# ratt-ru/pfb-clean

Measured on AMD Instinct MI355X. Metric: PCG matvecs/sec (FFT-conv A^H A apply), 4k x 4k x 8-band cube, higher is better.
Workload: dtype f32; 1 GPU; 4096x4096x8-band cube PCG (hessian_psf + Tikhonov, M = x/sigmainv, tol=0, minit=maxit=20); nx_psf=8192, bands_per_gpu=8, parallelism=band-shard x1, allreduce_hook=False

## Files before the change

pfb_clean_amd/csrc/fft_pow2.hpp:

```cpp
#pragma once
#include "common.hpp"
#include <type_traits>

namespace pfb {

constexpr int ilog2(int n) { return n <= 1 ? 0 : 1 + ilog2(n >> 1); }
constexpr int imin(int a, int b) { return a < b ? a : b; }

constexpr int rmax_of(int E) { return E < 16 ? E : 16; }

template <int N, int E, int P> struct PassRadix { static constexpr int R = imin(rmax_of(E), N / P); };

template <int N, int E, int P>
struct PtwOffset {
    static constexpr int RM = rmax_of(E);
    static constexpr int prev = P / RM;
    static constexpr int value = (P <= RM) ? 0 : PtwOffset<N, E, (P / RM < 1 ? 1 : P / RM)>::value + 4 * prev;
};
template <int N, int E> struct PtwOffset<N, E, 1> { static constexpr int value = 0; };

template <int N, int E>
constexpr int ptw_total() {
    int tot = 0;
    for (int P = rmax_of(E); P < N; P *= rmax_of(E)) tot += 4 * P;
// ... 59 lines not shown

template <typename T, bool INV, int m>
__device__ __forceinline__ cplx<T> mul_w16(cplx<T> a) {
    constexpr T c = T(0.92387953251128675612818318939678828682L);
    constexpr T s = T(0.38268343236508977172845998403039886676L);
    constexpr T h = T(0.70710678118654752440084436210484903928L);
    constexpr int mm = m & 15;
    if constexpr (mm == 0) return a;
    else if constexpr (mm == 4) return rot90<T, INV>(a);
    else if constexpr (mm == 8) return cplx<T>(-a.x, -a.y);
    else if constexpr (mm == 12) return rot90<T, !INV>(a);
    else if constexpr (mm == 2)  return h * (INV ? mul_1pi(a) : mul_1mi(a));
    else if constexpr (mm == 14) return h * (INV ? mul_1mi(a) : mul_1pi(a));
    else if constexpr (mm == 6)  return (-h) * (INV ? mul_1mi(a) : mul_1pi(a));
    else if constexpr (mm == 10) return (-h) * (INV ? mul_1pi(a) : mul_1mi(a));
    else {
        constexpr T wr = (mm == 1) ? c : (mm == 3) ? s : (mm == 5) ? -s : (mm == 7) ? -c : (mm == 9) ? -c
                       : (mm == 11) ? -s : (mm == 13) ? s : c;
        constexpr T wi = (mm == 1) ? s : (mm == 3) ? c : (mm == 5) ? c : (mm == 7) ? s : (mm == 9) ? -s
                       : (mm == 11) ? -c : (mm == 13) ? -c : -s;
        const T wy = INV ? wi : -wi;
        return a * cplx<T>(wr, wy);
    }
}

template <typename T, bool INV, int R> struct Dft;

template <typename T, bool INV> struct Dft<T, INV, 2> {
    __device__ __forceinline__ static void run(cplx<T> (&u)[2]) { dft2<T, INV>(u[0], u[1]); }
};
template <typename T, bool INV> struct Dft<T, INV, 4> {
    __device__ __forceinline__ static void run(cplx<T> (&u)[4]) { dft4<T, INV>(u[0], u[1], u[2], u[3]); }
};
template <typename T, bool INV> struct Dft<T, INV, 8> {
    __device__ __forceinline__ static void run(cplx<T> (&u)[8]) {
        dft4<T, INV>(u[0], u[2], u[4], u[6]);
        dft4<T, INV>(u[1], u[3], u[5], u[7]);
        u[3] = mul_w16<T, INV, 2>(u[3]);
        u[7] = mul_w16<T, INV, 6>(u[7]);
        cplx<T> x[8];
#pragma unroll
        for (int k1 = 0; k1 < 4; ++k1) {
            const cplx<T> p = u[2 * k1], q = u[2 * k1 + 1];
            if (k1 == 2) {
                x[k1] = addrot<INV>(p, q);
                x[k1 + 4] = addrot<!INV>(p, q);
            } else {
                x[k1] = p + q;
                x[k1 + 4] = p - q;
            }
        }
#pragma unroll
        for (int k = 0; k < 8; ++k) u[k] = x[k];
    }
};
template <typename T, bool INV> struct Dft<T, INV, 16> {
    __device__ __forceinline__ static void run(cplx<T> (&u)[16]) {
        dft4<T, INV>(u[0], u[4], u[8], u[12]);
        dft4<T, INV>(u[1], u[5], u[9], u[13]);
        dft4<T, INV>(u[2], u[6], u[10], u[14]);
        dft4<T, INV>(u[3], u[7], u[11], u[15]);
        u[5] = mul_w16<T, INV, 1>(u[5]);   u[6] = mul_w16<T, INV, 2>(u[6]);   u[7] = mul_w16<T, INV, 3>(u[7]);
        u[9] = mul_w16<T, INV, 2>(u[9]);   u[10] = mul_w16<T, INV, 4>(u[10]); u[11] = mul_w16<T, INV, 6>(u[11]);
        u[13] = mul_w16<T, INV, 3>(u[13]); u[14] = mul_w16<T, INV, 6>(u[14]); u[15] = mul_w16<T, INV, 9>(u[15]);
        dft4<T, INV>(u[0], u[1], u[2], u[3]);
        dft4<T, INV>(u[4], u[5], u[6], u[7]);
        dft4<T, INV>(u[8], u[9], u[10], u[11]);
        dft4<T, INV>(u[12], u[13], u[14], u[15]);
        cplx<T> t;
        t = u[1];  u[1] = u[4];   u[4] = t;
        t = u[2];  u[2] = u[8];   u[8] = t;
        t = u[3];  u[3] = u[12];  u[12] = t;
        t = u[6];  u[6] = u[9];   u[9] = t;
        t = u[7];  u[7] = u[13];  u[13] = t;
        t = u[11]; u[11] = u[14]; u[14] = t;
    }
};

struct NoPassHook {
    template <typename K> __device__ __forceinline__ void operator()(K) const {}
};
template <int K> using PassIdx = std::integral_constant<int, K>;

template <typename T, int N, int E, bool WAVE = false, int DBOFF = 0, bool SQTW = false, bool SEQX = false>
struct RegFft {
    static_assert((N & (N - 1)) == 0 && (E & (E - 1)) == 0 && N >= E, "power-of-two sizes");
    static_assert(!WAVE || N / E <= 64, "wave-local exchange needs the group inside one wave");
    __device__ __forceinline__ static void sync() {
        if constexpr (WAVE) __builtin_amdgcn_fence(__ATOMIC_ACQ_REL, "wavefront");
        else __syncthreads();
    }
    static constexpr int TPB = N / E;
    static constexpr int RM = rmax_of(E);
    static constexpr int LDS_ELEMS = N + N / (RM < (128 / (int)sizeof(cplx<T>)) ? RM : (128 / (int)sizeof(cplx<T>)));
    static constexpr int PTW = ptw_total<N, E>();
    static constexpr int PTWC = ptw_total<N, E>() / 4;

    __device__ __forceinline__ static int pad(int i) { return i + (i >> 4); }
    static constexpr int cpad(int c) { return c + (c >> 4); }

    static constexpr int CB = (int)sizeof(cplx<T>);
    static constexpr int SLOTS = 128 / CB;
    template <int P, int R>
    static constexpr int cxpad(int c) {
        if (P == 1) return c + c / SLOTS;
        if (P >= SLOTS) return c;
        return c + (c / (P * R)) * P;
    }
    template <int P, int R>
    __device__ __forceinline__ static int xpad(int c) { return cxpad<P, R>(c); }

    template <bool INV, int P>
    __device__ __forceinline__ static void butterflies(cplx<T> (&v)[E], int t, const cplx<T>* __restrict__ ptw) {
        constexpr int R = PassRadix<N, E, P>::R;
        constexpr int NB = E / R;
#pragma unroll
        for (int q = 0; q < NB; ++q) {
            cplx<T> u[R];
#pragma unroll
            for (int r = 0; r < R; ++r) u[r] = v[q + r * NB];
            if constexpr (P > 1) {
                const int k = (t + TPB * q) & (P - 1);
                const cplx<T>* tb = ptw + (SQTW ? PtwOffset<N, E, P>::value / 4 : PtwOffset<N, E, P>::value) + k;
                cplx<T> w1 = tb[0], w2, w4, w8;
                if constexpr (SQTW) {
                    if constexpr (R > 2) w2 = w1 * w1;
                    if constexpr (R > 4) w4 = w2 * w2;
                    if constexpr (R > 8) w8 = w4 * w4;
                } else {
                    if constexpr (R > 2) w2 = tb[P];
                    if constexpr (R > 4) w4 = tb[2 * P];
                    if constexpr (R > 8) w8 = tb[3 * P];
                }
                auto tw = [](cplx<T> a, cplx<T> w) { return INV ? mulc(a, w) : a * w; };
                u[1] = tw(u[1], w1);
                if constexpr (R > 2) {
                    u[2] = tw(u[2], w2);
                    const cplx<T> w3 = w1 * w2;
                    u[3] = tw(u[3], w3);
                    if constexpr (R > 4) {
                        u[4] = tw(u[4], w4);
                        const cplx<T> w7 = w3 * w4;
                        u[7] = tw(u[7], w7);
                        if constexpr (R > 8) { u[11] = tw(u[11], w3 * w8); u[15] = tw(u[15], w7 * w8); }
                        const cplx<T> w5 = w1 * w4;
                        u[5] = tw(u[5], w5);
                        if constexpr (R > 8) u[13] = tw(u[13], w5 * w8);
                        const cplx<T> w6 = w2 * w4;
                        u[6] = tw(u[6], w6);
                        if constexpr (R > 8) {
                            u[14] = tw(u[14], w6 * w8);
                            u[8] = tw(u[8], w8);
                            u[9] = tw(u[9], w1 * w8);
                            u[10] = tw(u[10], w2 * w8);
                            u[12] = tw(u[12], w4 * w8);
                        }
                    }
                }
            }
            Dft<T, INV, R>::run(u);
#pragma unroll
            for (int r = 0; r < R; ++r) v[q + r * NB] = u[r];
        }
    }

    template <bool INV, int P, int NV, int XCH = 0, int K = 0, typename Hook = NoPassHook>
    __device__ __forceinline__ static void pass(cplx<T> (&v)[NV][E], cplx<T>* lds_in, int t,
                                                const cplx<T>* __restrict__ ptw, const Hook& hook = Hook()) {
        constexpr int R = PassRadix<N, E, P>::R;
        constexpr int NB = E / R;
        hook(PassIdx<K>{});
#pragma unroll
        for (int n = 0; n < NV; ++n) butterflies<INV, P>(v[n], t, ptw);
        if constexpr (P * R < N) {
            cplx<T>* lds = (DBOFF > 0 && (XCH & 1) == 0) ? lds_in + DBOFF : lds_in;
            if constexpr (SEQX) {
#pragma unroll
                for (int n = 0; n < NV; ++n) {
                    sync();
#pragma unroll
                    for (int q = 0; q < NB; ++q) {
                        const int i = t + TPB * q;
                        const int k = i & (P - 1);
                        cplx<T>* wp = lds + xpad<P, R>((i - k) * R + k);
#pragma unroll
                        for (int s = 0; s < R; ++s) wp[cxpad<P, R>(s * P)] = v[n][q + s * NB];
                    }
                    sync();
                    const cplx<T>* rp = lds + xpad<P, R>(t);
#pragma unroll
                    for (int j = 0; j < E; ++j) v[n][j] = rp[cxpad<P, R>(TPB * j)];
                }
            } else {
            if constexpr (DBOFF == 0) sync();
#pragma unroll
            for (int q = 0; q < NB; ++q) {
                const int i = t + TPB * q;
                const int k = i & (P - 1);
                cplx<T>* wp = lds + xpad<P, R>((i - k) * R + k);
#pragma unroll
                for (int n = 0; n < NV; ++n) {
#pragma unroll
                    for (int s = 0; s < R; ++s) wp[n * LDS_ELEMS + cxpad<P, R>(s * P)] = v[n][q + s * NB];
                }
            }
            sync();
            const cplx<T>* rp = lds + xpad<P, R>(t);
#pragma unroll
            for (int n = 0; n < NV; ++n) {
#pragma unroll
                for (int j = 0; j < E; ++j) v[n][j] = rp[n * LDS_ELEMS + cxpad<P, R>(TPB * j)];
            }
            }
            pass<INV, P * R, NV, XCH + 1, K + 1, Hook>(v, lds_in, t, ptw, hook);
        }
    }

    template <bool INV, int NV, int X0 = 0, typename Hook = NoPassHook>
    __device__ __forceinline__ static void runN(cplx<T> (&v)[NV][E], cplx<T>* lds, int t,
                                                const cplx<T>* __restrict__ ptw, const Hook& hook = Hook()) {
        pass<INV, 1, NV, X0, 0, Hook>(v, lds, t, ptw, hook);
    }
    template <int P = 1> static constexpr int nxch() {
        constexpr int R = PassRadix<N, E, P>::R;
        if constexpr (P * R < N) return 1 + nxch<P * R>();
        else return 0;
    }
    static constexpr int NPASS = nxch<1>() + 1;
    template <bool INV, typename Hook = NoPassHook>
    __device__ __forceinline__ static void run(cplx<T> (&v)[E], cplx<T>* lds, int t,
                                               const cplx<T>* __restrict__ ptw, const Hook& hook = Hook()) {
        pass<INV, 1, 1, 0, 0, Hook>(reinterpret_cast<cplx<T>(&)[1][E]>(v), lds, t, ptw, hook);
    }
};

}
```

pfb_clean_amd/csrc/fftconv_pow2.hip:

```cpp
#include "conv_plan.hpp"
#include "fft_pow2.hpp"
#include <vector>
#include <cstdlib>

#ifndef PFB_POW2_PART
#define PFB_POW2_PART 0
#endif
#define PFB_POW2_COL  (PFB_POW2_PART != 1)
#define PFB_POW2_REST (PFB_POW2_PART != 2)

namespace pfb {

#ifndef PFB_STAMP
#define PFB_STAMP 0
#endif
#if PFB_STAMP
#define PFB_STAMP_ITS 4
#define PFB_STAMP_FIRST 2
static __device__ unsigned long long* g_stamp_buf = nullptr;
#define STAMP(KID, it, slot)                                                                              \
    do {                                                                                                  \
        const unsigned _si = (unsigned)((it) - PFB_STAMP_FIRST);                                          \
        if (threadIdx.x == 0 && g_stamp_buf && _si < PFB_STAMP_ITS && blockIdx.x < 1024)                  \
            g_stamp_buf[(((size_t)(KID) * 1024 + blockIdx.x) * PFB_STAMP_ITS + _si) * 16 + (slot)] = wall_clock64(); \
    } while (0)
#else
#define STAMP(KID, it, slot) do { (void)(it); } while (0)
#endif

template <typename T> struct FastCfg;
template <> struct FastCfg<float>  { static constexpr int ECOL = 8; static constexpr int EROWMAX = 32; static constexpr int WCOL = 4; static constexpr int NVB = 2; };
template <> struct FastCfg<double> { static constexpr int ECOL = 8; static constexpr int EROWMAX = 16; static constexpr int WCOL = 2; static constexpr int NVB = 1; };

template <typename T, int L, int E, int GMAX> constexpr int row_groups();
template <typename T, int L, bool INVK> struct RowCfg {
    static constexpr int EMAX = sizeof(T) == 4 ? (INVK ? (L == 4096 ? 16 : 8) : 16) : 8;
    static constexpr int E = (L / 64 < 8) ? 8 : (L / 64 > EMAX ? EMAX : L / 64);
    static constexpr int TPB = L / E;
    static constexpr bool WAVE = TPB <= 64;
    static constexpr int GMAX = INVK ? 4 : 8;
};
template <typename T, int L> struct InvDb {
    using C = RowCfg<T, L, true>;
    static constexpr int G = row_groups<T, L, C::E, C::GMAX>();
    static constexpr int STRIDE = RegFft<T, L, C::E>::LDS_ELEMS + 4;
    static constexpr bool ON = (size_t)(2 * G * STRIDE + L) * sizeof(cplx<T>) + 384 <= (size_t)152 * 1024;
    static constexpr int OFF = ON ? G * STRIDE : 0;
};

constexpr int LDS_BUDGET = 152 * 1024;

constexpr int COL_E4_MAXH = 1024;
template <typename T, int H> constexpr int ecol() { return (H >= 8192 && sizeof(T) == 8) ? 16 : (H <= COL_E4_MAXH && H >= 64 ? 4 : FastCfg<T>::ECOL); }

template <typename T, int L, int E, int GMAX>
constexpr int row_groups() {
    constexpr int TPB = L / E;
    int G = 256 / TPB > GMAX ? 256 / TPB : GMAX;
    const int stride = RegFft<T, L, E>::LDS_ELEMS + 4;
    while (G > 1 && (G * TPB > 1024 || (size_t)G * stride * sizeof(cplx<T>) + 384 > LDS_BUDGET)) G /= 2;
    return G;
}
template <int H, int E>
constexpr int col_groups() { return (H / E) >= 256 ? 1 : 256 / (H / E); }
constexpr int ECOLX = 8;

template <typename T, int NVB> struct alignas(16) Blk { cplx<T> c[NVB]; };
template <typename T, int NVB>
__device__ __forceinline__ Blk<T, NVB> loadb(const cplx<T>* src) {
    return *reinterpret_cast<const Blk<T, NVB>*>(src);
}
template <typename T, int NVB>
__device__ __forceinline__ Blk<T, NVB> loadb_nt(const cplx<T>* src) {
    typedef float v4f __attribute__((ext_vector_type(4)));
    static_assert(sizeof(Blk<T, NVB>) == 16, "16-byte blocks");
    const v4f v = __builtin_nontemporal_load(reinterpret_cast<const v4f*>(src));
    Blk<T, NVB> b;
    __builtin_memcpy(&b, &v, 16);
    return b;
}

template <typename T, int NVB>
__device__ __forceinline__ void storeb(cplx<T>* dst, const Blk<T, NVB>& b) {
    *reinterpret_cast<Blk<T, NVB>*>(dst) = b;
}

template <typename P>
__device__ __forceinline__ P* opaque(P* p) {
    asm volatile("" : "+v"(p));
    return p;
}

__device__ __forceinline__ int launder(int v) {
    asm volatile("" : "+v"(v));
    return v;
}

template <typename T>
__device__ __forceinline__ cplx<T> root32(int k) {
    constexpr T C[9] = {T(1), T(0.98078528040323044912618223613423903697L), T(0.92387953251128675612818318939678828682L),
                        T(0.83146961230254523707878837761790575673L), T(0.70710678118654752440084436210484903928L),
                        T(0.55557023301960222474283081394853287438L), T(0.38268343236508977172845998403039886676L),
                        T(0.19509032201612826784828486847702224093L), T(0)};
    auto cs = [&](int q) -> T {
        q &= 31;
        return q <= 8 ? C[q] : q <= 16 ? -C[16 - q] : q <= 24 ? -C[q - 16] : C[32 - q];
    };
    return cplx<T>(cs(k), -cs(k - 8));
}

template <int G>
__device__ __forceinline__ int xcd_row_group(int bx, int nbx) {
    constexpr int SH = 8 / G;
    if constexpr (SH > 1) {
        if (nbx % (8 * SH) == 0) {
            const int q = bx / (8 * SH), rem = bx % (8 * SH);
            return SH * (q * 8 + (rem & 7)) + (rem >> 3);
        }
    }
    return bx;
}

struct FastDims {
    int nx, ny, M;
    size_t T_band, psf_band;
    size_t xpitch, xband;
};

__host__ __device__ inline void block_of_bin(int v, int L, int nvb, int* blk, int* c) {
    const int m = v >> 1;
    const int nbe = (L + nvb) / nvb;
    *blk = ((v & 1) ? nbe : 0) + m / nvb;
    *c = m % nvb;
}
inline int fast_nblocks(int L, int nvb) { return (L + nvb) / nvb + L / nvb; }
__host__ __device__ inline size_t psf_off(int blk, int u, int c, int H, int nvb, int four) {
// ... 195 lines not shown
        const cplx<T>* c0 = col_of(act ? item : 0);
#pragma unroll
        for (int j = 0; j < E; ++j) {
            if (act) an[j] = loadb<T, NVB>(c0 + NVB * TPB * j);
            else {
#pragma unroll
                for (int c = 0; c < NVB; ++c) an[j].c[c] = cplx<T>(0, 0);
            }
        }
        {
            const cplx<T>* pe0 = psf_of(act ? item : 0);
#pragma unroll
            for (int j = 0; j < E; ++j) q[j] = NT ? loadb_nt<T, NVB>(pe0 + NVB * TPB * j) : loadb<T, NVB>(pe0 + NVB * TPB * j);
        }
    }
    __syncthreads();
#pragma unroll 1
    for (int it = 0; it < niter; ++it, item = item_of(it)) {
        STAMP(1, it, 0);
        const bool active = item < nitems;
        cplx<T>* col = col_of(active ? item : 0);
        const cplx<T>* pe = psf_of(active ? item : 0);
        const cplx<T>* po = pe + (size_t)H * NVB;
        const int nxt = item_of(it + 1);
        const bool nact = nxt < nitems;
        const cplx<T>* cn = col_of(nact ? nxt : (active ? item : 0));
        const cplx<T>* pen = psf_of(nact ? nxt : (active ? item : 0));
        cplx<T> vv[NVB][E], aw[NVB][E];
#pragma unroll
        for (int j = 0; j < E; ++j) {
#pragma unroll
            for (int c = 0; c < NVB; ++c) { vv[c][j] = an[j].c[c]; aw[c][j] = vv[c][j] * tw[j]; }
        }
        auto ld_an = [&](auto k, int base) {
            constexpr int K = decltype(k)::value;
            constexpr int CNT = E / 2;
#pragma unroll
            for (int j = (K * CNT) / NP; j < ((K + 1) * CNT) / NP; ++j)
                an[base + j] = loadb<T, NVB>(cn + NVB * TPB * (base + j));
        };
        STAMP(1, it, 1);
        F::template runN<false, NVB, 0>(vv, lds, t, ltw, [&](auto k) { ld_an(k, 0); });
        STAMP(1, it, 2);
#pragma unroll
        for (int j = 0; j < E; ++j) {
#pragma unroll
            for (int c = 0; c < NVB; ++c) vv[c][j] = vv[c][j] * q[j].c[c];
        }
        STAMP(1, it, 3);
        F::template runN<true, NVB, X1>(vv, lds, t, ltw, [&](auto k) {
            constexpr int K = decltype(k)::value;
#pragma unroll
            for (int j = (K * E) / NP; j < ((K + 1) * E) / NP; ++j) q[j] = NT ? loadb_nt<T, NVB>(po + NVB * TPB * j) : loadb<T, NVB>(po + NVB * TPB * j);
        });
        STAMP(1, it, 4);
        cplx<T> ev[NVB][E];
#pragma unroll
        for (int j = 0; j < E; ++j) {
#pragma unroll
            for (int c = 0; c < NVB; ++c) { ev[c][j] = vv[c][j]; vv[c][j] = aw[c][j]; }
        }
        F::template runN<false, NVB, 0>(vv, lds, t, ltw, [&](auto k) { ld_an(k, E / 2); });
        STAMP(1, it, 5);
#pragma unroll
        for (int j = 0; j < E; ++j) {
#pragma unroll
            for (int c = 0; c < NVB; ++c) vv[c][j] = vv[c][j] * q[j].c[c];
        }
        STAMP(1, it, 6);
        F::template runN<true, NVB, X1>(vv, lds, t, ltw, [&](auto k) {
            constexpr int K = decltype(k)::value;
#pragma unroll
            for (int j = (K * E) / NP; j < ((K + 1) * E) / NP; ++j) q[j] = NT ? loadb_nt<T, NVB>(pen + NVB * TPB * j) : loadb<T, NVB>(pen + NVB * TPB * j);
        });
        STAMP(1, it, 7);
        if (active) {
#pragma unroll
            for (int j = 0; j < E; ++j) {
                Blk<T, NVB> o;
#pragma unroll
                for (int c = 0; c < NVB; ++c) o.c[c] = ev[c][j] + mulc(vv[c][j], tw[j]);
                storeb<T, NVB>(col + NVB * TPB * j, o);
            }
        }
        STAMP(1, it, 8);
    }
}

template <typename T, int H, int E>
struct ColX {
    static constexpr int HS = H / 2;
    using F = RegFft<T, HS, E, false, 0, true>;
    static constexpr int NVB = FastCfg<T>::NVB;
    static constexpr int GC = col_groups<HS, E>();
    static constexpr int NT = GC * F::TPB;
    static constexpr int XB = NVB * F::LDS_ELEMS;
    static constexpr int PTWP = (F::PTWC + 1) & ~1;
    static constexpr size_t LDS = sizeof(cplx<T>) * ((size_t)PTWP + F::TPB + (size_t)GC * XB + (size_t)NT * E * NVB);
    static_assert(E == 8, "root32: the twiddle constants are the 4E-th roots of unity");
};

template <typename T, int H, int E, bool NT = false>
__global__ void __launch_bounds__((ColX<T, H, E>::NT), 2)
k_col_pow2x(cplx<T>* __restrict__ Tw, const cplx<T>* __restrict__ psf_l,
            const cplx<T>* __restrict__ twP, const cplx<T>* __restrict__ ptwc,
            int nblk, int nitems, size_t T_band, size_t psf_band, int band0, int bstep) {
    using X = ColX<T, H, E>;
    using F = typename X::F;
    constexpr int NVB = X::NVB, HS = X::HS, TPB = F::TPB, GC = X::GC, NP = F::NPASS, NTH = X::NT;
    extern __shared__ __attribute__((aligned(16))) char smem[];
    const int g = threadIdx.x / TPB, t = threadIdx.x % TPB;
    cplx<T>* ltw = reinterpret_cast<cplx<T>*>(smem);
    cplx<T>* ltx = ltw + X::PTWP;
    cplx<T>* lds = ltx + TPB + (size_t)g * X::XB;
    Blk<T, NVB>* park = reinterpret_cast<Blk<T, NVB>*>(ltx + TPB + (size_t)GC * X::XB) + threadIdx.x;
    const int stride = gridDim.x * GC;
    const int niter = (nitems + stride - 1) / stride;

    for (int k = threadIdx.x; k < F::PTWC; k += NTH) ltw[k] = ptwc[k];
    for (int k = threadIdx.x; k < TPB; k += NTH) ltx[k] = twP[k];

    auto col_of = [&](int item) -> cplx<T>* {
        const int bl = item / nblk, blk = item - bl * nblk;
        return Tw + (size_t)(band0 + bstep * bl) * T_band + ((size_t)blk * H + t) * NVB;
    };
    auto psf_of = [&](int item) -> const cplx<T>* {
        const int bl = item / nblk, blk = item - bl * nblk;
        return psf_l + (size_t)(band0 + bstep * bl) * psf_band + ((size_t)blk * 2 * H + t) * NVB;
    };
    auto ldq = [&](const cplx<T>* p) __attribute__((always_inline)) { return NT ? loadb_nt<T, NVB>(p) : loadb<T, NVB>(p); };

    int item = blockIdx.x * GC + g;
    Blk<T, NVB> al[E], ah[E], q[E];
    {
        const bool act = item < nitems;
        const cplx<T>* c0 = col_of(act ? item : 0);
#pragma unroll
        for (int j = 0; j < E; ++j) {
            al[j] = loadb<T, NVB>(c0 + NVB * TPB * j);
            ah[j] = loadb<T, NVB>(c0 + NVB * (HS + TPB * j));
        }
    }
    __syncthreads();
#pragma unroll 1
    for (int it = 0; it < niter; ++it, item += stride) {
        const bool active = item < nitems;
        cplx<T>* col = col_of(active ? item : 0);
        const cplx<T>* ps = psf_of(active ? item : 0);
        const int nxt = item + stride;
        const bool nact = nxt < nitems;
        const cplx<T>* cn = col_of(nact ? nxt : (active ? item : 0));
        cplx<T> vv[NVB][E], ol[NVB][E];
        auto wt = [&]() __attribute__((always_inline)) { return ltx[launder(t)]; };
        auto mulq = [&]() __attribute__((always_inline)) {
#pragma unroll
            for (int j = 0; j < E; ++j) {
#pragma unroll
                for (int c = 0; c < NVB; ++c) vv[c][j] = vv[c][j] * q[j].c[c];
            }
        };
        auto qslice = [&](auto k, const cplx<T>* pq) __attribute__((always_inline)) {
            constexpr int K = decltype(k)::value;
#pragma unroll
            for (int j = (K * E) / NP; j < ((K + 1) * E) / NP; ++j) q[j] = ldq(pq + NVB * TPB * j);
        };
        auto fft_q = [&](const cplx<T>* pq) __attribute__((always_inline)) {
// ... 1088 lines not shown
    void* ptw_col;
    void* ptwc_col;
    void* ptw_row;
    void* ptw_row_inv;
    void* ptw_row_inv_p;
    void* twM;
    void* ptwc_row_fwd;
    int num_cu;
    void* ptwc_col_x;
    int col_x;
};
int pow2_col_set_attr(int dtype, int H);
int pow2_col_launch(pfb_conv_plan* p, const FastTables* ft, int band0, int nb, hipStream_t st);
int pow2_col_fwd_launch(pfb_conv_plan* p, const FastTables* ft, const void* Tq, int band, hipStream_t st);

#if PFB_POW2_REST
template <typename T, int N, int E>
static int upload_ptw(void** dev) {
    constexpr int n = ptw_total<N, E>();
    std::vector<cplx<T>> h(n > 0 ? n : 1);
    if (n > 0) fill_ptw<T, N, E>(h.data());
    PFB_HIP_CHECK(hipMalloc(dev, sizeof(cplx<T>) * h.size()));
    PFB_HIP_CHECK(hipMemcpy(*dev, h.data(), sizeof(cplx<T>) * h.size(), hipMemcpyHostToDevice));
    return PFB_OK;
}

template <typename T, int N, int E>
static int prep_ptw(void** dev) { return upload_ptw<T, N, E>(dev); }

template <typename T, int N, int E>
static int prep_ptw_compact(void** dev) {
    constexpr int n = ptw_total<N, E>() / 4;
    std::vector<cplx<T>> h(n > 0 ? n : 1);
    if (n > 0) fill_ptw_compact<T, N, E>(h.data());
    PFB_HIP_CHECK(hipMalloc(dev, sizeof(cplx<T>) * h.size()));
    PFB_HIP_CHECK(hipMemcpy(*dev, h.data(), sizeof(cplx<T>) * h.size(), hipMemcpyHostToDevice));
    return PFB_OK;
}

template <typename T, int L>
static int set_invp_attr() {
    constexpr int E = InvPE<T, L>::E;
    if constexpr (InvP<T, L, E>::OK) {
#define PFB_INVATTR(MODE, BM)                                                                           \
        PFB_HIP_CHECK(hipFuncSetAttribute((const void*)(k_row_inv_pow2p<T, L, E, MODE, BM>),             \
                                          hipFuncAttributeMaxDynamicSharedMemorySize, 160 * 1024))
        PFB_INVATTR(0, false); PFB_INVATTR(1, false); PFB_INVATTR(2, false);
        PFB_INVATTR(0, true);  PFB_INVATTR(1, true);  PFB_INVATTR(2, true);
        if constexpr (inv_pb_ok<T, L, E>()) {
            PFB_HIP_CHECK(hipFuncSetAttribute((const void*)(k_row_inv_pow2p<T, L, E, 2, false, true>),
                                              hipFuncAttributeMaxDynamicSharedMemorySize, 160 * 1024));
            PFB_HIP_CHECK(hipFuncSetAttribute((const void*)(k_row_inv_pow2p<T, L, E, 2, true, true>),
                                              hipFuncAttributeMaxDynamicSharedMemorySize, 160 * 1024));
        }
#undef PFB_INVATTR
    }
    return PFB_OK;
}

template <typename T, int L>
static int prep_fwdp(void** table) {
    if constexpr (FwdP<T, L>::OK) {
        int rc = prep_ptw_compact<T, L, FwdP<T, L>::EOK>(table);
        if (rc != PFB_OK) return rc;
        PFB_HIP_CHECK(hipFuncSetAttribute((const void*)(k_row_fwd_pow2q<T, L, false>),
                                          hipFuncAttributeMaxDynamicSharedMemorySize, 160 * 1024));
        PFB_HIP_CHECK(hipFuncSetAttribute((const void*)(k_row_fwd_pow2q<T, L, true>),
                                          hipFuncAttributeMaxDynamicSharedMemorySize, 160 * 1024));
    } else {
        PFB_HIP_CHECK(hipFuncSetAttribute((const void*)k_row_fwd_pow2<T, L, RowCfg<T, L, false>::E>,
                                          hipFuncAttributeMaxDynamicSharedMemorySize, 160 * 1024));
    }
    return PFB_OK;
}


template <typename T>
static int prep_tables(pfb_conv_plan* p, FastTables* ft) {
    const int H = p->nx, L = p->ny / 2;
    int rc = PFB_ERR_UNSUPPORTED;
    constexpr int lds_max = 160 * 1024;
    switch (H) {
#define X(NN) case NN: rc = prep_ptw<T, NN, ecol<T, NN>()>(&ft->ptw_col);                          \
        if (rc == PFB_OK) rc = prep_ptw_compact<T, NN, ecol<T, NN>()>(&ft->ptwc_col);             \
        if (rc == PFB_OK && NN == 8192) rc = prep_ptw_compact<T, 4096, ECOLX>(&ft->ptwc_col_x);         \
        if (rc == PFB_OK) rc = pow2_col_set_attr(p->dtype, NN); break;
        PFB_POW2_SIZES(X)
#undef X
        default: break;
    }
    if (rc != PFB_OK) return rc;
    rc = PFB_ERR_UNSUPPORTED;
    switch (L) {
#define X(NN) case NN: rc = prep_ptw<T, NN, RowCfg<T, NN, false>::E>(&ft->ptw_row);                   \
        if (rc == PFB_OK) rc = prep_ptw_compact<T, NN, RowCfg<T, NN, true>::E>(&ft->ptw_row_inv);    \
        if (rc == PFB_OK) { if (InvPE<T, NN>::E != RowCfg<T, NN, true>::E) rc = prep_ptw_compact<T, NN, InvPE<T, NN>::E>(&ft->ptw_row_inv_p); \
                            else ft->ptw_row_inv_p = ft->ptw_row_inv; }                            \
        if (rc == PFB_OK) PFB_HIP_CHECK(hipFuncSetAttribute((const void*)k_row_inv_pow2<T, NN, RowCfg<T, NN, true>::E>, \
            hipFuncAttributeMaxDynamicSharedMemorySize, lds_max));                                   \
        if (rc == PFB_OK) rc = set_invp_attr<T, NN>();                                               \
        if (rc == PFB_OK) rc = prep_fwdp<T, NN>(&ft->ptwc_row_fwd); break;
        PFB_POW2_SIZES(X)
#undef X
        default: break;
    }
    if (rc != PFB_OK) return rc;
    std::vector<cplx<T>> h(L);
    const long double two_pi = 6.283185307179586476925286766559005768L;
    for (int n = 0; n < L; ++n) {
        long double a = two_pi * (long double)n / (long double)p->ny;
        h[n] = cplx<T>((T)cosl(a), (T)(-sinl(a)));
    }
    PFB_HIP_CHECK(hipMalloc(&ft->twM, sizeof(cplx<T>) * L));
    PFB_HIP_CHECK(hipMemcpy(ft->twM, h.data(), sizeof(cplx<T>) * L, hipMemcpyHostToDevice));
    return PFB_OK;
}

template <typename T, int L>
static int rows_per_wg() { return row_groups<T, L, RowCfg<T, L, true>::E, RowCfg<T, L, true>::GMAX>(); }

bool pow2_supported(const pfb_conv_plan* p) {
    if (!is_pow2(p->nx) || !is_pow2(p->ny)) return false;
    if (p->P != 2 * p->nx || p->Q != 2 * p->ny) return false;
    if (p->nx < 64 || p->nx > 8192) return false;
    if (p->ny < 128 || p->ny > (p->dtype == PFB_F32 ? 16384 : 8192)) return false;
    return true;
}

int pow2_rows_per_wg(const pfb_conv_plan* p) {
    const int L = p->ny / 2;
    const bool f32 = p->dtype == PFB_F32;
    switch (L) {
#define X(NN) case NN: return f32 ? rows_per_wg<float, NN>() : rows_per_wg<double, NN>();
        PFB_POW2_SIZES(X)
#undef X
        default: return 0;
    }
}

int pow2_nblocks(const pfb_conv_plan* p) {
    return fast_nblocks(p->ny / 2, p->dtype == PFB_F32 ? FastCfg<float>::NVB : FastCfg<double>::NVB);
}
int pow2_nvb(const pfb_conv_plan* p) {
    return p->dtype == PFB_F32 ? FastCfg<float>::NVB : FastCfg<double>::NVB;
}

int pow2_prepare(pfb_conv_plan* p) {
    FastTables* ft = (FastTables*)calloc(1, sizeof(FastTables));
    PFB_REQUIRE(ft != nullptr, PFB_ERR_ALLOC, "pow2_prepare: host alloc failed");
    p->fast_tables = ft;
    int dev = 0;
    hipDeviceProp_t prop;
    if (hipGetDevice(&dev) == hipSuccess && hipGetDeviceProperties(&prop, dev) == hipSuccess)
        ft->num_cu = prop.multiProcessorCount;
    if (ft->num_cu <= 0) ft->num_cu = 256;
    ft->col_x = p->nx >= 8192 ? 1 : 0;
    return p->dtype == PFB_F32 ? prep_tables<float>(p, ft) : prep_tables<double>(p, ft);
}

void pow2_release(pfb_conv_plan* p) {
    FastTables* ft = (FastTables*)p->fast_tables;
    if (!ft) return;
    if (ft->ptw_col) (void)hipFree(ft->ptw_col);
    if (ft->ptwc_col) (void)hipFree(ft->ptwc_col);
    if (ft->ptwc_col_x) (void)hipFree(ft->ptwc_col_x);
    if (ft->ptw_row) (void)hipFree(ft->ptw_row);
    if (ft->ptw_row_inv_p && ft->ptw_row_inv_p != ft->ptw_row_inv) (void)hipFree(ft->ptw_row_inv_p);
// ... 19 lines not shown
int pow2_set_psfhat(pfb_conv_plan* p, const void* psfhat, hipStream_t st) {
    return p->dtype == PFB_F32 ? set_psfhat_t<float>(p, psfhat, st) : set_psfhat_t<double>(p, psfhat, st);
}

template <typename T, int L>
static void launch_row_fwd(pfb_conv_plan* p, const FastTables* ft, void* Tbuf, int band0, int nb, const void* x,
                           const void* beam, size_t xpitch, size_t xband, hipStream_t st);

template <typename T>
static int set_psf_t(pfb_conv_plan* p, const void* psf, void* psfhat_out, hipStream_t st) {
    const FastTables* ft = (const FastTables*)p->fast_tables;
    const int nx = p->nx, ny = p->ny, P = p->P, Q = p->Q, L = ny / 2;
    void* Tq = nullptr;
    if (hipMalloc(&Tq, sizeof(cplx<T>) * 4 * p->T_elems_per_band) != hipSuccess) {
        set_error("pow2_set_psf: device allocation failed (%zu B)", sizeof(cplx<T>) * 4 * p->T_elems_per_band);
        return PFB_ERR_ALLOC;
    }
    int rc = PFB_OK;
    for (int band = 0; band < p->nband && rc == PFB_OK; ++band) {
        const T* pb = (const T*)psf + (size_t)band * P * Q;
        for (int q = 0; q < 4; ++q) {
            const int a = q >> 1, b = q & 1;
            const T* src = pb + (size_t)((1 - a) * nx) * Q + (size_t)(1 - b) * ny;
            switch (L) {
#define X(NN) case NN: launch_row_fwd<T, NN>(p, ft, Tq, q, 1, src, nullptr, (size_t)Q, (size_t)0, st); break;
                PFB_POW2_SIZES(X)
#undef X
                default: set_error("pow2_set_psf: unsupported ny"); rc = PFB_ERR_UNSUPPORTED; break;
            }
        }
        if (rc == PFB_OK) rc = pow2_col_fwd_launch(p, ft, Tq, band, st);
    }
    if (rc == PFB_OK && psfhat_out) {
        const int nv = p->M + 1;
        dim3 grid((nv + 31) / 32, (P + 31) / 32, p->nband);
        hipLaunchKernelGGL((k_unrelayout_psf_pow2<T>), grid, dim3(256), 0, st, (const cplx<T>*)p->psf_l,
                           (cplx<T>*)psfhat_out, P, nv, L, FastCfg<T>::NVB, p->psf_elems_per_band, ft->col_x);
    }
    if (rc == PFB_OK && (hipGetLastError() != hipSuccess || hipStreamSynchronize(st) != hipSuccess)) {
        set_error("pow2_set_psf: kernel launch failed");
        rc = PFB_ERR_HIP;
    }
    (void)hipFree(Tq);
    return rc;
}

int pow2_set_psf(pfb_conv_plan* p, const void* psf, void* psfhat_out, hipStream_t st) {
    return p->dtype == PFB_F32 ? set_psf_t<float>(p, psf, psfhat_out, st) : set_psf_t<double>(p, psf, psfhat_out, st);
}

#endif

#if PFB_POW2_COL
template <typename T, int H>
static void launch_col(pfb_conv_plan* p, const FastTables* ft, int band0, int nb, hipStream_t st) {
    constexpr int E = ecol<T, H>();
    using F = RegFft<T, H, E>;
    constexpr int GC = col_groups<H, E>();
    const int nblk = fast_nblocks(p->ny / 2, FastCfg<T>::NVB);
    const int band_first = band0 + nb - 1;
    const bool psf_nt = sizeof(cplx<T>) * p->psf_elems_per_band * (size_t)nb >= ((size_t)200 << 20);
    if constexpr (H == 8192) {
        if (ft->col_x) {
            using CX = ColX<T, H, ECOLX>;
            using FX = typename CX::F;
            constexpr int GX = CX::GC;
            const int nitems = nblk * nb;
            const int wg_lds = (int)(((size_t)160 * 1024) / CX::LDS);
            int wg_per_cu = (8 * 64) / (GX * FX::TPB) > 0 ? (8 * 64) / (GX * FX::TPB) : 1;
            if (wg_per_cu > wg_lds) wg_per_cu = wg_lds > 0 ? wg_lds : 1;
            const int need = (nitems + GX - 1) / GX;
            const int grid = need < ft->num_cu * wg_per_cu ? need : ft->num_cu * wg_per_cu;
            const size_t ldsx = CX::LDS;
#define PFB_COLX(NTV)                                                                                          \
            hipLaunchKernelGGL((k_col_pow2x<T, H, ECOLX, NTV>), dim3(grid), dim3(GX * FX::TPB), ldsx, st,      \
                               (cplx<T>*)p->T, (const cplx<T>*)p->psf_l, (const cplx<T>*)p->twP,               \
                               (const cplx<T>*)ft->ptwc_col_x, nblk, nitems, p->T_elems_per_band,              \
                               p->psf_elems_per_band, band_first, -1)
            if (psf_nt) PFB_COLX(true); else PFB_COLX(false);
#undef PFB_COLX
            return;
        }
    }
    constexpr size_t lds = sizeof(cplx<T>) * (size_t)GC * FastCfg<T>::NVB * F::LDS_ELEMS;
    constexpr size_t tab = sizeof(cplx<T>) * (size_t)((F::PTWC + 1) & ~1);
    if constexpr (H >= 2048 && lds + tab <= (size_t)160 * 1024) {
        const int nitems = nblk * nb;
        constexpr int wg_per_cu = (8 * 64) / (GC * F::TPB) > 0 ? (8 * 64) / (GC * F::TPB) : 1;
        const int need = (nitems + GC - 1) / GC;
        const int grid = balanced_grid(need, ft->num_cu * wg_per_cu);
        constexpr bool db = wg_per_cu == 1 && 2 * lds + tab <= (size_t)160 * 1024;
#define PFB_COLP(NTV)                                                                                          \
        hipLaunchKernelGGL((k_col_pow2p<T, H, E, db, NTV>), dim3(grid), dim3(GC * F::TPB), (db ? 2 : 1) * lds + tab, st, \
                           (cplx<T>*)p->T, (const cplx<T>*)p->psf_l, (const cplx<T>*)p->twP,                   \
                           (const cplx<T>*)ft->ptwc_col, nblk, nitems, p->T_elems_per_band,                    \
                           p->psf_elems_per_band, band_first, -1)
        if (psf_nt) PFB_COLP(true); else PFB_COLP(false);
#undef PFB_COLP
        return;
    }
    hipLaunchKernelGGL((k_col_pow2<T, H, E>), dim3((nblk + GC - 1) / GC, nb), dim3(GC * F::TPB), lds, st,
                       (cplx<T>*)p->T, (const cplx<T>*)p->psf_l, (const cplx<T>*)p->twP,
                       (const cplx<T>*)ft->ptw_col, nblk, p->T_elems_per_band, p->psf_elems_per_band, band0);
}

template <typename T, int H>
static int col_set_attr() {
    constexpr int lds_max = 160 * 1024;
    constexpr int E = ecol<T, H>();
    PFB_HIP_CHECK(hipFuncSetAttribute((const void*)(k_col_pow2<T, H, E>), hipFuncAttributeMaxDynamicSharedMemorySize, lds_max));
    PFB_HIP_CHECK(hipFuncSetAttribute((const void*)(k_col_fwd_pow2<T, H, E>), hipFuncAttributeMaxDynamicSharedMemorySize, lds_max));
    using F = RegFft<T, H, E>;
    constexpr int GC = col_groups<H, E>();
    constexpr size_t lds = sizeof(cplx<T>) * (size_t)GC * FastCfg<T>::NVB * F::LDS_ELEMS;
    constexpr size_t tab = sizeof(cplx<T>) * (size_t)((F::PTWC + 1) & ~1);
    if constexpr (H >= 2048 && lds + tab <= (size_t)160 * 1024) {
        constexpr int wg_per_cu = (8 * 64) / (GC * F::TPB) > 0 ? (8 * 64) / (GC * F::TPB) : 1;
        constexpr bool db = wg_per_cu == 1 && 2 * lds + tab <= (size_t)160 * 1024;
        PFB_HIP_CHECK(hipFuncSetAttribute((const void*)(k_col_pow2p<T, H, E, db, false>), hipFuncAttributeMaxDynamicSharedMemorySize, lds_max));
        PFB_HIP_CHECK(hipFuncSetAttribute((const void*)(k_col_pow2p<T, H, E, db, true>), hipFuncAttributeMaxDynamicSharedMemorySize, lds_max));
    }
    if constexpr (H == 8192 || (H == 4096 && sizeof(T) == 8)) {
        PFB_HIP_CHECK(hipFuncSetAttribute((const void*)(k_col_pow2x<T, H, ECOLX, false>), hipFuncAttributeMaxDynamicSharedMemorySize, lds_max));
        PFB_HIP_CHECK(hipFuncSetAttribute((const void*)(k_col_pow2x<T, H, ECOLX, true>), hipFuncAttributeMaxDynamicSharedMemorySize, lds_max));
    }
    return PFB_OK;
}
template <typename T>
static int col_set_attr_t(int H) {
    switch (H) {
#define X(NN) case NN: return col_set_attr<T, NN>();
        PFB_POW2_SIZES(X)
#undef X
        default: set_error("pow2: unsupported nx"); return PFB_ERR_UNSUPPORTED;
    }
}
int pow2_col_set_attr(int dtype, int H) {
    return dtype == PFB_F32 ? col_set_attr_t<float>(H) : col_set_attr_t<double>(H);
}
template <typename T>
static int col_launch_t(pfb_conv_plan* p, const FastTables* ft, int band0, int nb, hipStream_t st) {
    switch (p->nx) {
#define X(NN) case NN: launch_col<T, NN>(p, ft, band0, nb, st); break;
        PFB_POW2_SIZES(X)
#undef X
        default: set_error("pow2_apply: unsupported nx"); return PFB_ERR_UNSUPPORTED;
    }
    return PFB_OK;
}
int pow2_col_launch(pfb_conv_plan* p, const FastTables* ft, int band0, int nb, hipStream_t st) {
    return p->dtype == PFB_F32 ? col_launch_t<float>(p, ft, band0, nb, st) : col_launch_t<double>(p, ft, band0, nb, st);
}
template <typename T, int H>
static void launch_col_fwd(pfb_conv_plan* p, const FastTables* ft, const void* Tq, int band, hipStream_t st) {
    constexpr int E = ecol<T, H>();
    using F = RegFft<T, H, E>;
    constexpr int GC = col_groups<H, E>();
    constexpr int NVB = FastCfg<T>::NVB;
    const int L = p->ny / 2;
    const int nblk = fast_nblocks(L, NVB), nbe = (L + NVB) / NVB;
    const size_t lds = sizeof(cplx<T>) * (size_t)GC * NVB * F::LDS_ELEMS;
    hipLaunchKernelGGL((k_col_fwd_pow2<T, H, E>), dim3((nblk + GC - 1) / GC), dim3(GC * F::TPB), lds, st,
                       (const cplx<T>*)Tq, (cplx<T>*)p->psf_l + (size_t)band * p->psf_elems_per_band,
                       (const cplx<T>*)p->twP, (const cplx<T>*)ft->ptw_col, nblk, nbe, p->T_elems_per_band, ft->col_x);
}
template <typename T>
static int col_fwd_launch_t(pfb_conv_plan* p, const FastTables* ft, const void* Tq, int band, hipStream_t st) {
    switch (p->nx) {
#define X(NN) case NN: launch_col_fwd<T, NN>(p, ft, Tq, band, st); break;
        PFB_POW2_SIZES(X)
#undef X
        default: set_error("pow2_set_psf: unsupported nx"); return PFB_ERR_UNSUPPORTED;
    }
    return PFB_OK;
}
int pow2_col_fwd_launch(pfb_conv_plan* p, const FastTables* ft, const void* Tq, int band, hipStream_t st) {
    return p->dtype == PFB_F32 ? col_fwd_launch_t<float>(p, ft, Tq, band, st) : col_fwd_launch_t<double>(p, ft, Tq, band, st);
}
#endif

#if PFB_POW2_REST

template <typename T, int L>
static void launch_row_fwd(pfb_conv_plan* p, const FastTables* ft, void* Tbuf, int band0, int nb, const void* x,
                           const void* beam, size_t xpitch, size_t xband, hipStream_t st) {
    FastDims d{p->nx, p->ny, p->M, p->T_elems_per_band, p->psf_elems_per_band, xpitch, xband};
    if constexpr (FwdP<T, L>::OK) {
        using FP = FwdP<T, L>;
        const int tiles_per_band = p->nx / FP::G, ntiles = tiles_per_band * nb;
        const int grid = ntiles < ft->num_cu * FP::WG_PER_CU ? ntiles : ft->num_cu * FP::WG_PER_CU;
        const long double a = 6.283185307179586476925286766559005768L / (2.0L * (long double)p->ny);
        const cplx<T> wq1((T)cosl(a), (T)(-sinl(a)));
#define PFB_FWDQ(BM)                                                                                              \
        hipLaunchKernelGGL((k_row_fwd_pow2q<T, L, BM>), dim3(grid), dim3(FP::NT), FP::LDS, st, (const T*)x,      \
                           (const T*)beam, (cplx<T>*)Tbuf, (const cplx<T>*)ft->twM,                              \
                           (const cplx<T>*)ft->ptwc_row_fwd, d, band0, tiles_per_band, ntiles, wq1)
        if (beam) PFB_FWDQ(true); else PFB_FWDQ(false);
#undef PFB_FWDQ
    } else {
// ... 128 lines not shown
```

Before: 437.5 cube-matvecs/s.

## Add single-column-per-thread column FFT-conv kernel for f32 4096-point columns

Adds a new column kernel for f32 with H=4096. Each thread pair splits the two interleaved 8-byte columns of a 16-byte block, so every thread handles one column with E=16 instead of a two-column register block. An LDS stride parameter lets the shared exchange interleave both columns, and the kernel uses double-buffered LDS, prefetches the next item's column and PSF data inside the FFT passes, and computes per-element twiddles from a 32nd-root table. The intent is to cut register pressure and raise occupancy, with more latency hidden by prefetching. The cost is more threads per block and narrower 8-byte global accesses in place of 16-byte ones.

```diff
diff --git a/pfb_clean_amd/csrc/fft_pow2.hpp b/pfb_clean_amd/csrc/fft_pow2.hpp
--- a/pfb_clean_amd/csrc/fft_pow2.hpp
+++ b/pfb_clean_amd/csrc/fft_pow2.hpp
@@ -165,7 +165,7 @@
 };
 template <int K> using PassIdx = std::integral_constant<int, K>;
 
-template <typename T, int N, int E, bool WAVE = false, int DBOFF = 0, bool SQTW = false, bool SEQX = false>
+template <typename T, int N, int E, bool WAVE = false, int DBOFF = 0, bool SQTW = false, bool SEQX = false, int LSTR = 1>
 struct RegFft {
     static_assert((N & (N - 1)) == 0 && (E & (E - 1)) == 0 && N >= E, "power-of-two sizes");
     static_assert(!WAVE || N / E <= 64, "wave-local exchange needs the group inside one wave");
@@ -265,14 +265,14 @@
                     for (int q = 0; q < NB; ++q) {
                         const int i = t + TPB * q;
                         const int k = i & (P - 1);
-                        cplx<T>* wp = lds + xpad<P, R>((i - k) * R + k);
-#pragma unroll
-                        for (int s = 0; s < R; ++s) wp[cxpad<P, R>(s * P)] = v[n][q + s * NB];
+                        cplx<T>* wp = lds + LSTR * xpad<P, R>((i - k) * R + k);
+#pragma unroll
+                        for (int s = 0; s < R; ++s) wp[LSTR * cxpad<P, R>(s * P)] = v[n][q + s * NB];
                     }
                     sync();
-                    const cplx<T>* rp = lds + xpad<P, R>(t);
-#pragma unroll
-                    for (int j = 0; j < E; ++j) v[n][j] = rp[cxpad<P, R>(TPB * j)];
+                    const cplx<T>* rp = lds + LSTR * xpad<P, R>(t);
+#pragma unroll
+                    for (int j = 0; j < E; ++j) v[n][j] = rp[LSTR * cxpad<P, R>(TPB * j)];
                 }
             } else {
             if constexpr (DBOFF == 0) sync();
@@ -280,19 +280,19 @@
             for (int q = 0; q < NB; ++q) {
                 const int i = t + TPB * q;
                 const int k = i & (P - 1);
-                cplx<T>* wp = lds + xpad<P, R>((i - k) * R + k);
+                cplx<T>* wp = lds + LSTR * xpad<P, R>((i - k) * R + k);
 #pragma unroll
                 for (int n = 0; n < NV; ++n) {
 #pragma unroll
-                    for (int s = 0; s < R; ++s) wp[n * LDS_ELEMS + cxpad<P, R>(s * P)] = v[n][q + s * NB];
+                    for (int s = 0; s < R; ++s) wp[LSTR * (n * LDS_ELEMS + cxpad<P, R>(s * P))] = v[n][q + s * NB];
                 }
             }
             sync();
-            const cplx<T>* rp = lds + xpad<P, R>(t);
+            const cplx<T>* rp = lds + LSTR * xpad<P, R>(t);
 #pragma unroll
             for (int n = 0; n < NV; ++n) {
 #pragma unroll
-                for (int j = 0; j < E; ++j) v[n][j] = rp[n * LDS_ELEMS + cxpad<P, R>(TPB * j)];
+                for (int j = 0; j < E; ++j) v[n][j] = rp[LSTR * (n * LDS_ELEMS + cxpad<P, R>(TPB * j))];
             }
             }
             pass<INV, P * R, NV, XCH + 1, K + 1, Hook>(v, lds_in, t, ptw, hook);
diff --git a/pfb_clean_amd/csrc/fftconv_pow2.hip b/pfb_clean_amd/csrc/fftconv_pow2.hip
--- a/pfb_clean_amd/csrc/fftconv_pow2.hip
+++ b/pfb_clean_amd/csrc/fftconv_pow2.hip
@@ -52,6 +52,9 @@
 
 constexpr int COL_E4_MAXH = 1024;
 template <typename T, int H> constexpr int ecol() { return (H >= 8192 && sizeof(T) == 8) ? 16 : (H <= COL_E4_MAXH && H >= 64 ? 4 : FastCfg<T>::ECOL); }
+
+template <typename T, int H> constexpr bool col_one() { return sizeof(T) == 4 && H == 4096; }
+template <typename T, int H> constexpr int ecolp() { return col_one<T, H>() ? 16 : ecol<T, H>(); }
 
 template <typename T, int L, int E, int GMAX>
 constexpr int row_groups() {
@@ -413,6 +416,109 @@
                 for (int c = 0; c < NVB; ++c) o.c[c] = ev[c][j] + mulc(vv[c][j], tw[j]);
                 storeb<T, NVB>(col + NVB * TPB * j, o);
             }
+        }
+        STAMP(1, it, 8);
+    }
+}
+
+template <typename T, int H, int E, bool DB, bool NT>
+__global__ void __launch_bounds__(FastCfg<T>::NVB * (H / E), 2)
+k_col_pow2s(cplx<T>* __restrict__ Tw, const cplx<T>* __restrict__ psf_l,
+            const cplx<T>* __restrict__ twP, const cplx<T>* __restrict__ ptwc,
+            int nblk, int nitems, size_t T_band, size_t psf_band, int band0, int bstep) {
+    constexpr int NVB = FastCfg<T>::NVB;
+    static_assert(NVB == 2 && sizeof(cplx<T>) == 8, "two 8-byte columns per 16-byte block");
+    constexpr int XB = NVB * RegFft<T, H, E>::LDS_ELEMS;
+    using F = RegFft<T, H, E, false, DB ? XB : 0, true, false, NVB>;
+    constexpr int X1 = (DB && (F::template nxch<1>() & 1)) ? 1 : 0;
+    constexpr int TPB = F::TPB;
+    constexpr int NP = F::NPASS;
+    static_assert(32 * TPB == 2 * H, "root32: w_P^(TPB j) must be a 32nd root of unity (P = 2 H)");
+    extern __shared__ __attribute__((aligned(16))) char smem[];
+    const int t = threadIdx.x >> 1, c = threadIdx.x & 1;
+    cplx<T>* ltw = reinterpret_cast<cplx<T>*>(smem);
+    cplx<T>* lds = ltw + ((F::PTWC + 1) & ~1) + c;
+    const int stride = gridDim.x;
+    const int niter = (nitems + stride - 1) / stride;
+
+    const cplx<T> wt = twP[t];
+    auto twj = [&](int j) __attribute__((always_inline)) { return j == 0 ? wt : wt * root32<T>(j); };
+    for (int k = threadIdx.x; k < F::PTWC; k += NVB * TPB) ltw[k] = ptwc[k];
+    auto ldq = [](const cplx<T>* src) __attribute__((always_inline)) {
+        if constexpr (NT) return cplx<T>(__builtin_nontemporal_load(reinterpret_cast<const v2f*>(src)));
+        else return *src;
+    };
+
+    auto col_of = [&](int item) -> cplx<T>* {
+        const int bl = item / nblk, blk = item - bl * nblk;
+        return Tw + (size_t)(band0 + bstep * bl) * T_band + ((size_t)blk * H + t) * NVB + c;
+    };
+    auto psf_of = [&](int item) -> const cplx<T>* {
+        const int bl = item / nblk, blk = item - bl * nblk;
+        return psf_l + (size_t)(band0 + bstep * bl) * psf_band + ((size_t)blk * 2 * H + t) * NVB + c;
+    };
+
+    auto item_of = [&](int it) -> int { return blockIdx.x + it * stride; };
+    int item = item_of(0);
+    cplx<T> an[E], q[E];
+    {
+        const bool act = item < nitems;
+        const cplx<T>* c0 = col_of(act ? item : 0);
+#pragma unroll
+        for (int j = 0; j < E; ++j) an[j] = act ? c0[NVB * TPB * j] : cplx<T>(0, 0);
+        const cplx<T>* pe0 = psf_of(act ? item : 0);
+#pragma unroll
+        for (int j = 0; j < E; ++j) q[j] = ldq(pe0 + NVB * TPB * j);
+    }
+    __syncthreads();
+#pragma unroll 1
+    for (int it = 0; it < niter; ++it, item = item_of(it)) {
+        STAMP(1, it, 0);
+        const bool active = item < nitems;
+        cplx<T>* col = col_of(active ? item : 0);
+        const cplx<T>* po = psf_of(active ? item : 0) + (size_t)H * NVB;
+        const int nxt = item_of(it + 1);
+        const bool nact = nxt < nitems;
+        const cplx<T>* cn = col_of(nact ? nxt : (active ? item : 0));
+        const cplx<T>* pen = psf_of(nact ? nxt : (active ? item : 0));
+        cplx<T> vv[1][E], aw[E];
+#pragma unroll
+        for (int j = 0; j < E; ++j) { vv[0][j] = an[j]; aw[j] = vv[0][j] * twj(j); }
+        auto ld_an = [&](auto k, int base) {
+            constexpr int K = decltype(k)::value;
+            constexpr int CNT = E / 2;
+#pragma unroll
+            for (int j = (K * CNT) / NP; j < ((K + 1) * CNT) / NP; ++j) an[base + j] = cn[NVB * TPB * (base + j)];
+        };
+        STAMP(1, it, 1);
+        F::template runN<false, 1, 0>(vv, lds, t, ltw, [&](auto k) { ld_an(k, 0); });
+        STAMP(1, it, 2);
+#pragma unroll
+        for (int j = 0; j < E; ++j) vv[0][j] = vv[0][j] * q[j];
+        STAMP(1, it, 3);
+        F::template runN<true, 1, X1>(vv, lds, t, ltw, [&](auto k) {
+            constexpr int K = decltype(k)::value;
+#pragma unroll
+            for (int j = (K * E) / NP; j < ((K + 1) * E) / NP; ++j) q[j] = ldq(po + NVB * TPB * j);
+        });
+        STAMP(1, it, 4);
+        cplx<T> ev[E];
+#pragma unroll
+        for (int j = 0; j < E; ++j) { ev[j] = vv[0][j]; vv[0][j] = aw[j]; }
+        F::template runN<false, 1, 0>(vv, lds, t, ltw, [&](auto k) { ld_an(k, E / 2); });
+        STAMP(1, it, 5);
+#pragma unroll
+        for (int j = 0; j < E; ++j) vv[0][j] = vv[0][j] * q[j];
+        STAMP(1, it, 6);
+        F::template runN<true, 1, X1>(vv, lds, t, ltw, [&](auto k) {
+            constexpr int K = decltype(k)::value;
+#pragma unroll
+            for (int j = (K * E) / NP; j < ((K + 1) * E) / NP; ++j) q[j] = ldq(pen + NVB * TPB * j);
+        });
+        STAMP(1, it, 7);
+        if (active) {
+#pragma unroll
+            for (int j = 0; j < E; ++j) col[NVB * TPB * j] = ev[j] + mulc(vv[0][j], twj(j));
         }
         STAMP(1, it, 8);
     }
@@ -1667,7 +1773,7 @@
     constexpr int lds_max = 160 * 1024;
     switch (H) {
 #define X(NN) case NN: rc = prep_ptw<T, NN, ecol<T, NN>()>(&ft->ptw_col);                          \
-        if (rc == PFB_OK) rc = prep_ptw_compact<T, NN, ecol<T, NN>()>(&ft->ptwc_col);             \
+        if (rc == PFB_OK) rc = prep_ptw_compact<T, NN, ecolp<T, NN>()>(&ft->ptwc_col);             \
         if (rc == PFB_OK && NN == 8192) rc = prep_ptw_compact<T, 4096, ECOLX>(&ft->ptwc_col_x);         \
         if (rc == PFB_OK) rc = pow2_col_set_attr(p->dtype, NN); break;
         PFB_POW2_SIZES(X)
@@ -1853,6 +1959,22 @@
             return;
         }
     }
+    if constexpr (col_one<T, H>()) {
+        using FS = RegFft<T, H, ecolp<T, H>()>;
+        constexpr int NVB = FastCfg<T>::NVB;
+        constexpr size_t ldss = sizeof(cplx<T>) * ((size_t)((FS::PTWC + 1) & ~1) + 2 * (size_t)NVB * FS::LDS_ELEMS);
+        static_assert(ldss <= (size_t)160 * 1024, "k_col_pow2s: LDS");
+        const int nitems = nblk * nb;
+        constexpr int wg_per_cu = (8 * 64) / (NVB * FS::TPB);
+        const int grid = balanced_grid(nitems, ft->num_cu * wg_per_cu);
+#define PFB_COLS(NTV)                                                                                          \
+        hipLaunchKernelGGL((k_col_pow2s<T, H, ecolp<T, H>(), true, NTV>), dim3(grid), dim3(NVB * FS::TPB), ldss, st, \
+                           (cplx<T>*)p->T, (const cplx<T>*)p->psf_l, (const cplx<T>*)p->twP,                   \
+                           (const cplx<T>*)ft->ptwc_col, nblk, nitems, p->T_elems_per_band,                    \
+                           p->psf_elems_per_band, band_first, -1)
+        if (psf_nt) PFB_COLS(true); else PFB_COLS(false);
+#undef PFB_COLS
+    } else {
     constexpr size_t lds = sizeof(cplx<T>) * (size_t)GC * FastCfg<T>::NVB * F::LDS_ELEMS;
     constexpr size_t tab = sizeof(cplx<T>) * (size_t)((F::PTWC + 1) & ~1);
     if constexpr (H >= 2048 && lds + tab <= (size_t)160 * 1024) {
@@ -1873,6 +1995,7 @@
     hipLaunchKernelGGL((k_col_pow2<T, H, E>), dim3((nblk + GC - 1) / GC, nb), dim3(GC * F::TPB), lds, st,
                        (cplx<T>*)p->T, (const cplx<T>*)p->psf_l, (const cplx<T>*)p->twP,
                        (const cplx<T>*)ft->ptw_col, nblk, p->T_elems_per_band, p->psf_elems_per_band, band0);
+    }
 }
 
 template <typename T, int H>
@@ -1885,7 +2008,10 @@
     constexpr int GC = col_groups<H, E>();
     constexpr size_t lds = sizeof(cplx<T>) * (size_t)GC * FastCfg<T>::NVB * F::LDS_ELEMS;
     constexpr size_t tab = sizeof(cplx<T>) * (size_t)((F::PTWC + 1) & ~1);
-    if constexpr (H >= 2048 && lds + tab <= (size_t)160 * 1024) {
+    if constexpr (col_one<T, H>()) {
+        PFB_HIP_CHECK(hipFuncSetAttribute((const void*)(k_col_pow2s<T, H, ecolp<T, H>(), true, false>), hipFuncAttributeMaxDynamicSharedMemorySize, lds_max));
+        PFB_HIP_CHECK(hipFuncSetAttribute((const void*)(k_col_pow2s<T, H, ecolp<T, H>(), true, true>), hipFuncAttributeMaxDynamicSharedMemorySize, lds_max));
+    } else if constexpr (H >= 2048 && lds + tab <= (size_t)160 * 1024) {
         constexpr int wg_per_cu = (8 * 64) / (GC * F::TPB) > 0 ? (8 * 64) / (GC * F::TPB) : 1;
         constexpr bool db = wg_per_cu == 1 && 2 * lds + tab <= (size_t)160 * 1024;
         PFB_HIP_CHECK(hipFuncSetAttribute((const void*)(k_col_pow2p<T, H, E, db, false>), hipFuncAttributeMaxDynamicSharedMemorySize, lds_max));
```

After: 432.7 cube-matvecs/s. 1.1% lower.
